# firstBusiness/mathmap

Hardware: AMD Instinct MI355X
Metric: Mpixels/sec (mandelbrot @8192x8192) (higher is better)
Workload: dtype f32

## Files before the change

### mathmap_amd/csrc/hipgen.cpp

```cpp
#include <cmath>
#include <cstdio>
#include <cstdlib>
#include <cstring>
#include <map>
#include <set>
#include <sstream>
#include <stdexcept>

#include "front.h"
#include "hipgen_internal.h"

namespace mm {
namespace hipgen {

std::optional<int> env_int(const char *name) {
    const char *e = getenv(name);
    return e ? std::optional<int>(atoi(e)) : std::nullopt;
}

std::string vname(const Value *v) {
    char buf[64];
    snprintf(buf, sizeof buf, "v%d_%d", v->var->id, v->index);
    return buf;
}
// ... 581 lines not shown
                ok = true;
                bool any_row = false;
                for (const Primary &p : r.args) {
                    ok = ok && operand_ok(p) && (p.kind != Primary::Val || p.value->index < 0 || row_scalar(p.value->var->type));
                    any_row = any_row || (p.kind == Primary::Val && rows.count(p.value));
                }
                ok = ok && any_row && strncmp(r.op->cname, "USERVAL_", 8) != 0;
            }
            if (!ok) continue;
            cand.push_back(s);
            rows.insert(s->lhs);
        }
        std::set<Value *> used;
        for (bool changed = true; changed;) {
            changed = false;
            for (Stmt *s : cand) s->in_pixel = !rows.count(s->lhs);
            std::vector<Value *> defs;
            used.clear();
            collect_values(code.body, PIXEL, defs, used);
            for (int i = 0; i < 4; ++i) used.insert(code.result[i]);
            for (Stmt *s : cand) {
                if (!rows.count(s->lhs)) continue;
                bool drop = used.count(s->lhs) && s->lhs->var->type == Ty::Complex;
                if (s->rhs.kind == Rhs::Prim) drop = drop || !rows.count(s->rhs.prim.value);
                for (const Primary &p : s->rhs.args)
                    drop = drop || (p.kind == Primary::Val && p.value->index >= 0 && !p.value->hoisted && !rows.count(p.value));
                if (drop) { rows.erase(s->lhs); changed = true; }
            }
        }
        bool expensive = false;
        for (Stmt *s : cand)
            expensive = expensive || (rows.count(s->lhs) && s->rhs.kind == Rhs::Op && row_expensive(s->rhs.op->cname));
        for (Stmt *s : cand) if (rows.count(s->lhs) && used.count(s->lhs)) row_transfer.push_back(s->lhs);
        if (!expensive || row_transfer.empty() || row_transfer.size() > 24) {
            for (Stmt *s : cand) s->in_pixel = true;
            row_transfer.clear();
            return;
        }
        for (Stmt *s : cand)
            if (rows.count(s->lhs)) { s->in_row = true; s->in_pixel = false; s->lhs->row_const = true; }
        ks.row_values = (int)row_transfer.size();
        ks.rows_name = "mm_rows";
    }
    void transfer_loads(const std::set<Value *> *only, const char *ind = "  ") {
        for (Value *v : transfer_order)
            if (!only || only->count(v))
                out << ind << "const " << ctype(v->var) << " " << vname(v) << " = *(const " << ctype(v->var) << " *)(XY + " << transfer_off[v] << ");\n";
    }
    void row_loads(const std::string &ind, const char *row) {
        for (size_t k = 0; k < row_transfer.size(); ++k) {
            Value *v = row_transfer[k];
            const std::string at = "A.rowtab[" + std::to_string(k) + " * A.num_rows + " + row + "]";
            out << ind << "const " << ctype(v->var) << " " << vname(v) << " = "
                << (v->var->type == Ty::Int ? "__float_as_int(" + at + ")" : at) << ";\n";
        }
    }

    void analyze_and_layout() {
        find_natives(code.body);
        ks.native_sites = (int)ks.natives.size();
        bool any_in_loop = false;
        for (const NativeCall &nc : ks.natives) any_in_loop = any_in_loop || nc.in_loop;
        NativeCall dynamic_entry;
        dynamic_entry.dynamic = true;
        if (any_in_loop) ks.natives.insert(ks.natives.end(), MM_NATIVE_DYN_CALLS, dynamic_entry);
        ks.direct_native = find_direct_native();
        find_row_slice();
        collect_values(code.body, PROLOGUE, pro_defs, pro_uses);
        collect_values(code.body, PIXEL, pix_defs, pix_uses);
        collect_values(code.body, ROWS, row_defs, row_uses);
        for (Value *v : row_uses) if (v && v->hoisted) pix_uses.insert(v);
        for (int i = 0; i < 4; ++i) pix_uses.insert(code.result[i]);
        std::set<Value *> pix_def_set(pix_defs.begin(), pix_defs.end());
        for (Value *v : row_transfer) pix_def_set.insert(v);
        int off = 0;
        for (NativeCall &nc : ks.natives) {
            nc.record_offset = off;
            off += MM_NATIVE_REC_BYTES;
        }
        if (!ks.natives.empty()) {
            ks.native_ctr_offset = off;
            off += 16;
        }
        for (Value *v : pro_defs) {
            if (!pix_uses.count(v) || pix_def_set.count(v) || transfer_off.count(v)) continue;
            int sz = type_size(v->var);
            int align = sz >= 8 ? 8 : 4;
            off = (off + align - 1) / align * align;
            transfer_off[v] = off;
            transfer_order.push_back(v);
            off += sz;
        }
        if (ks.native_sites < (int)ks.natives.size())
            each_stmt(code.body, [&](const Stmt *s) {
                if (s->kind != Stmt::While || !s->hoisted || !s->in_pixel) return true;
                off = (off + 3) / 4 * 4;
                dual_base_off[s] = off;
                off += 4;
                return false;
            });
        ks.xy_bytes = (off + 15) / 16 * 16;
        if (ks.xy_bytes == 0) ks.xy_bytes = 16;
        ks.has_prologue = !pro_defs.empty();
        for (Value *v : pix_uses)
            if (v && v->index >= 0 && !pix_def_set.count(v) && !transfer_off.count(v))
                throw CompileError("internal: value " + vname(v) + " used in the pixel kernel but defined nowhere");
        pixel_stats(code.body, pixel_stmts, pixel_fetches);
    }

    void run() {
        analyze_and_layout();
        emit_options();
        emit_preludes();
        emit_functions();
        if (pair) pair->emit_helpers();
        emit_prologue_kernel();
        if (ks.row_values > 0) emit_rows_kernel();
        if (opt.sampled) emit_sampled_pixel_kernel();
        else if (opt.shutter) emit_shutter_pixel_kernel();
        else emit_pixel_kernel();
        ks.source = out.str();
        if (opt.variant()) {
            std::string text, key;
            clip_kernel_source(ks, &text, &key);
            ks.source = std::move(text);
            ks.clip_splices.clear();
        }
        ks.key = text_key(ks.source);
        ks.wrapping_ints = opt.edge_x >= 2 || opt.edge_y >= 2;
    }

    void emit_options() {
        int tw = knobs.tile_w.value_or(opt.tile_w);
        if (tw != 8 && tw != 16 && tw != 32 && tw != 64 && tw != 128 && tw != 256) tw = auto_tile_w();
        ks.tile_w = tw;
        ks.tile_h = 256 / tw;
        out << "#define MM_NT_STORE " << knobs.nt_store.value_or(pixel_fetches > 0) << "\n";
        ks.xcd_order = knobs.xcd_order.value_or(2);
        out << "#define MM_XCD_ORDER " << ks.xcd_order << "\n";
        if (knobs.pair_masks) out << "#define MM_PAIR_MASKS " << *knobs.pair_masks << "\n";
        if (knobs.no_same_taps) out << "#define MM_NO_SAME_TAPS 1\n";
        if (knobs.no_outside_shortcut) out << "#define MM_NO_OUTSIDE_SHORTCUT 1\n";
        out << "#define MM_INTERSAMPLE " << opt.intersample << "\n";
        out << "#define MM_SUPERSAMPLING " << opt.supersampling << "\n";
        out << "#define MM_EDGE_X " << opt.edge_x << "\n#define MM_EDGE_Y " << opt.edge_y << "\n";
        if (opt.pixel_inc > 1) out << "#define MM_PIXEL_INC " << opt.pixel_inc << "\n";
        out << "#define MM_TILE_W " << ks.tile_w << "\n#define MM_TILE_H " << ks.tile_h << "\n";
        ks.unroll = opt.unroll > 0 ? opt.unroll : auto_unroll();
        if (opt.variant()) ks.unroll = 1;
        else if (opt.unroll <= 0 && !knobs.unroll && ks.row_values == 0 && ks.natives.empty())
            pair = make_pair_mode(PairEnv{out, code, opt, knobs, pix_defs, pixel_stmts, pixel_fetches,
                                          [this](const Primary &p) { return prim(p, PIXEL); },
                                          [this](const Stmt *s) { return rhs(s->rhs, PIXEL, s, s->lhs->var); },
                                          [this](const Value *v) { return value_visible(v, PIXEL); }});
        if (pair) ks.unroll = 2;
        ks.pair_mode = pair != nullptr;
        ks.pair_exit = pair && pair->exit_driven();
        out << "#define MM_UNROLL " << ks.unroll << "\n";
        out << "#define MM_NATIVE_REC_BYTES " << (int)MM_NATIVE_REC_BYTES << "\n#define MM_NATIVE_DYN_CALLS " << (int)MM_NATIVE_DYN_CALLS << "\n";
    }

    void emit_preludes() {
        out << "#define MMF_FN static __device__ __forceinline__\n#define MMF_CONST_TABLE static __device__ const\n"
               "#define MMG_FN static __device__\n"
               "#define MMF_FMA(a, b, c) __builtin_fma((a), (b), (c))\n#define MMF_RINT(a) __builtin_rint((a))\n"
               "#define MMF_FABSF(a) __builtin_fabsf((a))\n#define MMF_FABS(a) __builtin_fabs((a))\n"
               "#define MMF_SIN_SLOW(a) sin((a))\n#define MMF_COS_SLOW(a) cos((a))\n"
               "#define MMF_LDEXP(a, e) __builtin_ldexp((a), (e))\n#define MMF_EXP_SLOW(a) exp((a))\n#define MMF_LOG_SLOW(a) log((a))\n"
               "#define MMF_POW_SLOW(a, b) pow((a), (b))\n"
               "#define MMF_ASINH_SLOW(a) asinh((a))\n#define MMF_ACOSH_SLOW(a) acosh((a))\n"
               "#define MMF_SQRT(a) __builtin_sqrt((a))\n#define MMF_HYPOT_SLOW(a, b) hypot((a), (b))\n"
               "#define MMQ_FN static __device__ __forceinline__\n#define MMQ_TABLE static __device__ const\n"
               "#define MMQ_FMA(a, b, c) __builtin_fma((a), (b), (c))\n#define MMQ_SQRT(a) sqrt((a))\n"
               "#define MMQ_SQRTF(a) sqrtf((a))\n"
            << device_fastmath_prelude() << "\n";
        out << device_prelude() << "\n";
        bool noise = uses_noise(code.body);
        for (auto &fn : (fn_root ? fn_root : &code)->functions) noise = noise || uses_noise(fn->body);
        if (noise) {
            if (!noise_table_text())
                throw CompileError("the noise builtins need libnoise's gradient table, which was not available when this "
                                   "library was built (see tools/extract_noise_table.py)");
            out << noise_table_text() << device_noise_prelude() << "\n";
        }
        out << R"(
MM_DEV mm_image mm_closure_image(const mm_args &A, int closure_id) {
    mm_image im; im.idx = closure_id < 0 ? -1 : -2 - closure_id; im.pw = A.img_width; im.ph = A.img_height;
    im.xf = im.yf = 1.0f; im.resized = 0; return im;
}
struct mm_narg_t { int kind; int i; float f; mm_image img; };
MM_DEV mm_narg_t mm_narg(int v) { mm_narg_t a; a.kind = 0; a.i = v; a.f = (float)v; a.img = mm_null_image(); return a; }
MM_DEV mm_narg_t mm_narg(float v) { mm_narg_t a; a.kind = 1; a.i = (int)v; a.f = v; a.img = mm_null_image(); return a; }
MM_DEV mm_narg_t mm_narg(double v) { return mm_narg((float)v); }
MM_DEV mm_narg_t mm_narg(mm_image v) { mm_narg_t a; a.kind = 2; a.i = v.idx; a.f = 0.0f; a.img = v; return a; }
// Records a native-filter call for the host (which runs the filter's kernels between
// the prologue and the pixel kernel) and returns the handle of its result float map.
// ctr[0] counts the calls of this frame in the order they are made (the host runs them in that order).
MM_DEV mm_image mm_native_call(const mm_args &A, char *rec, int *ctr, int k, int nargs, mm_narg_t a0, mm_narg_t a1, mm_narg_t a2, mm_narg_t a3) {
    int *hdr = (int *)rec;
    hdr[0] = 1; hdr[1] = k; hdr[2] = nargs; hdr[3] = ctr[0]++;
    mm_narg_t *args = (mm_narg_t *)(rec + 16);
    args[0] = a0; args[1] = a1; args[2] = a2; args[3] = a3;
    mm_image im; im.idx = A.native_slot_base + k; im.pw = A.render_width; im.ph = A.render_height;
    im.xf = im.yf = 1.0f; im.resized = 0;
    return im;
}
// The same for a call site inside a loop: every call takes the next of the MM_NATIVE_DYN_CALLS dynamic entries behind
// the `sites' call sites (record, result slot); one call too many raises ctr[2] and the host refuses the frame.
MM_DEV mm_image mm_native_call_in_loop(const mm_args &A, char *dyn, int *ctr, int site, int sites, int nargs, mm_narg_t a0, mm_narg_t a1,
                                       mm_narg_t a2, mm_narg_t a3) {
    int n = ctr[1]++;
    if (n >= MM_NATIVE_DYN_CALLS) { ctr[2] = 1; n = MM_NATIVE_DYN_CALLS - 1; }
    mm_image im = mm_native_call(A, dyn + n * MM_NATIVE_REC_BYTES, ctr, site, nargs, a0, a1, a2, a3);
    im.idx = A.native_slot_base + sites + n;
    return im;
}
// (float) frame column / row of the pixel being evaluated (render_image's per-pixel loop, builtins.c:324-333)
#define __colF ((float)(col + A.region_x))
#define __rowF ((float)(rl + A.first_row))
#define MM_INTERNALS \
    const float t = A.t; const float R = A.R; const int frame = A.frame; \
    const int __canvasPixelW = A.img_width, __canvasPixelH = A.img_height; \
    const int __renderPixelW = A.render_width, __renderPixelH = A.render_height; \
    (void)t; (void)R; (void)frame; (void)__canvasPixelW; (void)__canvasPixelH; (void)__renderPixelW; (void)__renderPixelH;
)";
        if (ks.native_sites < (int)ks.natives.size())
            out << R"(// The pixel slice's side of a loop that runs in both slices: its n-th call from an in-loop site is the prologue's n-th.
MM_DEV mm_image mm_native_result_in_loop(const mm_args &A, int &n, int sites) {
    mm_image im; im.idx = A.native_slot_base + sites + (n < MM_NATIVE_DYN_CALLS ? n : MM_NATIVE_DYN_CALLS - 1); ++n;
    im.pw = A.render_width; im.ph = A.render_height; im.xf = im.yf = 1.0f; im.resized = 0;
    return im;
}
)";
    }

    void emit_functions() {
        FilterCode &root = fn_root ? *fn_root : code;
        if (root.functions.empty()) return;
        out << "#ifndef MM_MAX_CALL_DEPTH\n#define MM_MAX_CALL_DEPTH " << knobs.max_call_depth.value_or(16)
            << "\n#endif\n"
               "struct mm_uvarg { int i; float f; color_t c; mm_image img; };\n";
        auto head = [](size_t k) {
            return "template <int MM_D> __device__ __noinline__ mm_tup<4> mm_filter_" + std::to_string(k) +
                   "(const mm_args &A, const mm_uvarg *UV, float x, float y, float t, int col, int rl, unsigned &mm_rand_ctr)";
        };
        for (size_t k = 0; k < root.functions.size(); ++k) out << head(k) << ";\n";
        for (size_t k = 0; k < root.functions.size(); ++k) {
            FilterCode &fn = *root.functions[k];
            Generator g(fn, opt, knobs);
            g.fn_root = &root;
            g.in_function = true;
            std::vector<Value *> defs;
            std::set<Value *> uses;
            g.collect_values(fn.body, PIXEL, defs, uses);
            out << "// filter_" << (fn.filter ? fn.filter->name : "") << "\n" << head(k) << " {\n"
                   "  mm_tup<4> rt;\n  rt.v[0] = rt.v[1] = rt.v[2] = rt.v[3] = 0.0f;\n"
                   "  if constexpr (MM_D >= MM_MAX_CALL_DEPTH) { return rt; } else {\n"
                   "  const float R = A.R; const int frame = 0;      // new_template.c.in:379: filter_$name has `int frame = 0`\n"
                   "  const int __canvasPixelW = A.img_width, __canvasPixelH = A.img_height;\n"
                   "  const int __renderPixelW = A.render_width, __renderPixelH = A.render_height;\n"
                   "  (void)R; (void)frame; (void)__canvasPixelW; (void)__canvasPixelH; (void)__renderPixelW; (void)__renderPixelH;\n";
            g.decls(defs, "  ");
            g.stmts(fn.body, PIXEL, "  ");
            out << g.out.str();
            for (int i = 0; i < 4; ++i) out << "  rt.v[" << i << "] = " << g.prim(Primary::V(fn.result[i]), PIXEL) << ";\n";
            out << "  return rt;\n  }\n}\n";
        }
    }

    void emit_prologue_kernel() {
        ks.prologue_uses_time = hoisted_uses_time(code.body);
        ks.prologue_name = "mm_prologue";
        ks.pixel_name = "mm_pixels";
        auto tables = [](const std::string &first) {
            return "  {\n    const int gid = blockIdx.x * 256 + threadIdx.x;\n"
                   "    if (" + first + "gid < A.region_width) A.xtab[gid] = CALC_VIRTUAL_X(gid + A.region_x, A.frame_render_width, A.sampling_offset_x);\n"
                   "    if (" + first + "gid < A.num_rows) A.ytab[gid] = CALC_VIRTUAL_Y(A.first_row + gid, A.frame_render_height, A.sampling_offset_y);\n"
                   "    if (gid != 0) return;\n  }\n";
        };
        const std::string sampled_tables =
            "  {\n    const int gid = blockIdx.x * 256 + threadIdx.x;\n"
            "    if (fi == 0 && gid < A.region_width) {\n"
            "      A.xtab[gid] = CALC_VIRTUAL_X(gid + A.region_x, A.frame_render_width, A.sampling_offset_x);\n"
            "      for (int mm_a = 0; mm_a < S.gx; ++mm_a)\n"
            "        S.xtabs[mm_a * A.region_width + gid] = CALC_VIRTUAL_X(gid + A.region_x, A.frame_render_width, S.offs[mm_a]);\n"
            "    }\n"
            "    if (fi == 0 && gid < A.num_rows) {\n"
            "      A.ytab[gid] = CALC_VIRTUAL_Y(A.first_row + gid, A.frame_render_height, A.sampling_offset_y);\n"
            "      for (int mm_b = 0; mm_b < S.gy; ++mm_b)\n"
            "        S.ytabs[mm_b * A.num_rows + gid] = CALC_VIRTUAL_Y(A.first_row + gid, A.frame_render_height, S.offs[MM_SAMPLE_GRID_MAX + mm_b]);\n"
            "    }\n"
            "    if (gid != 0) return;\n  }\n";
        const std::string clip_head =
            opt.sampled ? std::string(clip_prelude()) + sampled_prelude() + KERNEL +
                              "mm_prologue_clip(mm_args A, char *XY, const mm_clip C, const mm_sampled S) {\n  MM_CLIP_ENTRY\n" + sampled_tables
                        : (ks.natives.empty() ? clip_prelude() : clip_prelude_natives()) + KERNEL +
                              "mm_prologue_clip(mm_args A, char *XY, const mm_clip C) {\n  MM_CLIP_ENTRY\n" + tables("fi == 0 && ");
        emit(KERNEL + "mm_prologue(mm_args A, char *XY) {\n" + tables(""), clip_head);
        out << "  MM_INTERNALS\n";
        if (!(fn_root ? fn_root : &code)->functions.empty()) out << "  const int col = 0, rl = 0; unsigned mm_rand_ctr = 0; (void)col; (void)rl; (void)mm_rand_ctr;\n";
        decls(pro_defs, "  ", true);
        if (!ks.natives.empty()) {
            for (const NativeCall &nc : ks.natives) out << "  *(int *)(XY + " << nc.record_offset << ") = 0;\n";
            out << "  { int *mm_ctr = (int *)(XY + " << ks.native_ctr_offset << "); mm_ctr[0] = mm_ctr[1] = mm_ctr[2] = mm_ctr[3] = 0; }\n";
        }
        stmts(code.body, PROLOGUE, "  ");
        for (Value *v : transfer_order)
// ... 337 lines not shown
```

### mathmap_amd/csrc/hipgen_internal.h

```cpp
#pragma once
#include <functional>
#include <memory>
#include <optional>
#include <ostream>
#include <string>
#include <vector>

#include "hipgen.h"

namespace mm {
namespace hipgen {

enum Slice { PROLOGUE, PIXEL, ROWS };

std::optional<int> env_int(const char *name);
struct Knobs {
    std::optional<int> unroll = env_int("MMHIP_UNROLL");
    std::optional<int> tile_w = env_int("MMHIP_TILE_W");
    std::optional<int> single_pixel = env_int("MMHIP_SINGLE_PIXEL");
    std::optional<int> pair = env_int("MMHIP_PAIR");
    bool pair_debug = env_int("MMHIP_PAIR_DEBUG").has_value();
    std::optional<int> pair_masks = env_int("MMHIP_PAIR_MASKS");
    std::optional<int> pair_exit = env_int("MMHIP_PAIR_EXIT");
    std::optional<int> pair_exit_tail = env_int("MMHIP_PAIR_EXIT_TAIL");
    std::optional<int> pair_pack = env_int("MMHIP_PAIR_PACK");
    std::optional<int> pair_peel = env_int("MMHIP_PAIR_PEEL");
    std::optional<int> pair_fma2 = env_int("MMHIP_PAIR_FMA2");
    std::optional<int> pair_step = env_int("MMHIP_PAIR_STEP");
    bool pair_no_uniform = env_int("MMHIP_PAIR_NO_UNIFORM").has_value();
    std::optional<int> nt_store = env_int("MMHIP_NT_STORE");
    std::optional<int> xcd_order = env_int("MMHIP_XCD_ORDER");
    std::optional<int> waves_per_eu = env_int("MMHIP_WAVES_PER_EU");
    bool no_fetched_result = env_int("MMHIP_NO_FETCHED_RESULT").has_value();
    bool no_same_taps = env_int("MMHIP_NO_SAME_TAPS").has_value();
    bool no_outside_shortcut = env_int("MMHIP_NO_OUTSIDE_SHORTCUT").has_value();
    std::optional<int> frame_hot = env_int("MMHIP_FRAME_HOT");
    bool no_row_slice = env_int("MMHIP_NO_ROW_SLICE").has_value();
    std::optional<int> max_call_depth = env_int("MMHIP_MAX_CALL_DEPTH");
};

std::string vname(const Value *v);
std::string ctype(const CompVar *v);
int type_size(const CompVar *v);
std::string float_literal(float f);
const char *libm_name(const char *cname, bool f32);
bool is_truth_op(const char *cname);
bool is_pow2_divisor(float c);
bool nonneg_or_nan(const Value *v, int depth);
const Primary *sqrt_less_pow2(const Rhs &r, float *kk);

struct PairEnv {
    std::ostream &out;
    FilterCode &code;
    const KernelOptions &opt;
    const Knobs &knobs;
    const std::vector<Value *> &pix_defs;
    int pixel_stmts, pixel_fetches;
    std::function<std::string(const Primary &)> prim;
    std::function<std::string(const Stmt *)> rhs;
    std::function<bool(const Value *)> value_visible;
};
struct PairMode {
    virtual ~PairMode() {}
    virtual bool exit_driven() const = 0;
    virtual bool is_uniform(const Value *v) const = 0;
    virtual void emit_helpers() = 0;
    virtual void emit_pixel_loop(const std::string &ind) = 0;
};
std::unique_ptr<PairMode> make_pair_mode(const PairEnv &env);

}
}
```

### mathmap_amd/csrc/hipgen_pair.cpp

```cpp
#include <algorithm>
#include <cstdio>
#include <cstring>
#include <map>
#include <set>
#include <sstream>

#include "hipgen_internal.h"

namespace mm {
namespace hipgen {
namespace {

struct PairGen final : PairMode {
    PairEnv env;
    std::ostream &out;
    FilterCode &code;
    std::set<const Value *> defs;
    std::set<const Value *> bools;
    std::set<const Value *> uniform;
    int ids = 0;
    const bool exit = env.knobs.pair_exit.value_or(1) && env.knobs.pair_masks.value_or(1);
    const bool pack = exit && env.knobs.pair_pack.value_or(1);
    const Stmt *split_def = nullptr;
    bool split_leave = false;
    const bool fma2 = exit && env.knobs.pair_fma2.value_or(1) && env.knobs.pair_exit_tail.value_or(2) >= 2;
    struct Fuse { const Stmt *r, *d; Primary t, b; float k; bool keep_d; };
    std::map<const Stmt *, std::vector<Fuse>> fuse_plan;
    std::map<const Stmt *, const Fuse *> fusing;
    std::set<const Stmt *> fused_away;
    const bool step = fma2 && pack && !env.knobs.pair_peel.value_or(0) && env.knobs.pair_step.value_or(1);
    bool fast_step = false;
    std::vector<std::string> entry_masks;

    explicit PairGen(const PairEnv &e) : env(e), out(e.out), code(e.code) {}

    bool exit_driven() const override { return exit; }
    bool is_uniform(const Value *v) const override { return uniform.count(v) > 0; }

    static bool scalar_ty(Ty t) { return t == Ty::Int || t == Ty::Float; }
    static bool prim_ok(const Primary &p) {
        if (p.kind == Primary::IntConst || p.kind == Primary::FloatConst) return true;
        return p.kind == Primary::Val && scalar_ty(p.value->var->type);
    }
    static bool rhs_ok(const Rhs &r) {
        if (r.kind == Rhs::Prim) return prim_ok(r.prim);
        if (r.kind == Rhs::Internal) return r.internal == "x" || r.internal == "y";
        if (r.kind != Rhs::Op) return false;
        static const char *ok[] = {"ADD", "SUB", "MUL", "NEG", "DIV", "LESS", "LEQ", "EQ", "NOT", "sqrt"};
        bool found = false;
        for (const char *o : ok) found = found || !strcmp(r.op->cname, o);
        if (!found) return false;
        for (const Primary &a : r.args) if (!prim_ok(a)) return false;
        if (!strcmp(r.op->cname, "sqrt") && r.args[0].type() != Ty::Float) return false;
        if (!strcmp(r.op->cname, "NOT") && r.args[0].type() != Ty::Int) return false;
        return true;
    }
    bool block_ok(const Block &b) const {
        for (const Stmt *s : b) {
            if (!s->in_pixel) continue;
            switch (s->kind) {
                case Stmt::Assign:
                    if (!s->lhs || !scalar_ty(s->lhs->var->type) || !rhs_ok(s->rhs)) {
                        if (env.knobs.pair_debug)
                            fprintf(stderr, "pair mode: statement not covered (%s)\n",
                                    s->rhs.kind == Rhs::Op ? s->rhs.op->cname : s->rhs.kind == Rhs::Internal ? s->rhs.internal.c_str() : "rhs kind");
                        return false;
                    }
                    break;
                case Stmt::If:
                case Stmt::While:
                    if (s->cond.kind != Rhs::Prim || !prim_ok(s->cond.prim) || s->cond.prim.type() != Ty::Int) return false;
                    for (const Stmt *ph : s->phis) {
                        if (!ph->in_pixel) continue;
                        if (!scalar_ty(ph->lhs->var->type) || ph->rhs.kind != Rhs::Prim || ph->rhs2.kind != Rhs::Prim ||
                            !prim_ok(ph->rhs.prim) || !prim_ok(ph->rhs2.prim))
                            return false;
                    }
                    if (s->kind == Stmt::If ? !(block_ok(s->then_) && block_ok(s->else_)) : !block_ok(s->body)) return false;
                    break;
                default: break;
            }
        }
        return true;
    }
    bool eligible() const {
        if (!env.opt.fast_math_exact) return false;
        const bool force = env.knobs.pair.has_value();
        if (force && !*env.knobs.pair) return false;
        const int stmts = env.pixel_stmts;
        if (env.pixel_fetches || stmts < 4 || stmts > (force ? 400 : 40)) return false;
        const bool dbg = env.knobs.pair_debug;
        for (int i = 0; i < 4; ++i)
            if (!code.result[i] || !scalar_ty(code.result[i]->var->type)) {
                if (dbg) fprintf(stderr, "pair mode: result %d is not an int / float value\n", i);
                return false;
            }
        const bool ok = block_ok(code.body);
        if (dbg) fprintf(stderr, "pair mode: body %s (%d statements)\n", ok ? "covered" : "not covered", stmts);
        return ok;
    }

    template <class P> static bool truth_def(const Stmt *d, P operand) {
        if (d->kind == Stmt::Phi) return d->rhs.kind == Rhs::Prim && d->rhs2.kind == Rhs::Prim && operand(d->rhs.prim) && operand(d->rhs2.prim);
        if (d->kind != Stmt::Assign) return false;
        if (d->rhs.kind == Rhs::Prim) return operand(d->rhs.prim);
        return d->rhs.kind == Rhs::Op && is_truth_op(d->rhs.op->cname);
    }
    static bool const_is_bool(const Value *v, int depth) {
        if (!v || depth > 12 || v->var->type != Ty::Int) return false;
        if (v->index < 0) return true;
        return v->def && truth_def(v->def, [&](const Primary &p) {
            return p.kind == Primary::IntConst ? p.i == 0 || p.i == 1 : p.kind == Primary::Val && const_is_bool(p.value, depth + 1);
        });
    }
    bool prim_bool(const Primary &p) const {
        if (p.kind == Primary::IntConst) return p.i == 0 || p.i == 1;
        if (p.kind != Primary::Val) return false;
        if (p.value->index < 0) return p.value->var->type == Ty::Int;
        if (bools.count(p.value)) return true;
        return !defs.count(p.value) && const_is_bool(p.value, 0);
    }
    void infer_bools() {
        std::vector<const Stmt *> idefs;
        for (Value *v : env.pix_defs) {
            defs.insert(v);
            if (v->var->type == Ty::Int && v->def && v->def->lhs == v) idefs.push_back(v->def);
        }
        for (const Stmt *d : idefs) bools.insert(d->lhs);
        for (bool changed = true; changed;) {
            changed = false;
            for (const Stmt *d : idefs)
                if (bools.count(d->lhs) && !truth_def(d, [&](const Primary &p) { return prim_bool(p); })) { bools.erase(d->lhs); changed = true; }
        }
    }
    void uses_outside(const Block &b, const Stmt *skip, std::set<const Value *> &uses) const {
        auto use = [&](const Primary &p) { if (p.kind == Primary::Val) uses.insert(p.value); };
        auto use_rhs = [&](const Rhs &r) { if (r.kind == Rhs::Prim) use(r.prim); for (const Primary &a : r.args) use(a); };
        for (const Stmt *s : b) {
            if (!s->in_pixel) continue;
            if (s->kind == Stmt::Assign) use_rhs(s->rhs);
            if (s->kind == Stmt::If) {
                use_rhs(s->cond);
                uses_outside(s->then_, skip, uses);
                uses_outside(s->else_, skip, uses);
                for (const Stmt *ph : s->phis) if (ph->in_pixel) { use_rhs(ph->rhs); use_rhs(ph->rhs2); }
            }
            if (s->kind == Stmt::While) {
                for (const Stmt *ph : s->phis) if (ph->in_pixel) { use_rhs(ph->rhs); if (s != skip) use_rhs(ph->rhs2); }
                if (s != skip) { use_rhs(s->cond); uses_outside(s->body, skip, uses); }
            }
        }
    }

    std::string pbool(const Primary &p) {
        const std::string bu = exit ? "mm_xbu(" : "mm_bu(";
        if (p.kind == Primary::IntConst) return bu + (p.i ? "true)" : "false)");
        if (p.kind == Primary::Val && p.value->index < 0) return bu + "false)";
        if (uniform.count(p.value)) return "mm_bu((bool)u" + vname(p.value) + ")";
        if (bools.count(p.value)) return vname(p.value);
        if (fast_step && !defs.count(p.value)) {
            const std::string c = env.prim(p);
            size_t k = std::find(entry_masks.begin(), entry_masks.end(), c) - entry_masks.begin();
            if (k == entry_masks.size()) entry_masks.push_back(c);
            return "mm_ub" + std::to_string(k);
        }
        return "mm_tob(" + pprim(p, Ty::Int) + ")";
    }
    std::string pprim(const Primary &p, Ty want) {
        const char *w = want == Ty::Float ? "mm_vf(" : "mm_vi(";
        if (p.kind == Primary::IntConst) return std::string(w) + std::to_string(p.i) + ")";
        if (p.kind == Primary::FloatConst) return std::string(w) + float_literal(p.f) + "f)";
        if (p.value->index < 0) return std::string(w) + "0)";
        if (uniform.count(p.value))
            return std::string(w) + (p.value->var->type == Ty::Float ? "(float)u" : "(int)u") + vname(p.value) + ")";
        return std::string(w) + vname(p.value) + ")";
    }
    static Ty arith_ty(const Rhs &r) {
        for (const Primary &a : r.args) if (a.type() == Ty::Float) return Ty::Float;
        return Ty::Int;
    }
    std::string prhs(const Rhs &r, const Value *lhs) {
        const Ty lhs_ty = lhs->var->type;
        const bool as_bool = bools.count(lhs) > 0;
        if (r.kind == Rhs::Prim) return as_bool ? pbool(r.prim) : pprim(r.prim, lhs_ty);
// ... 585 lines not shown
                                << pval_as(ph->rhs2.prim, ph->lhs) << ");\n";
                    break;
                }
                case Stmt::While: while_loop(s, ind, mask); break;
                default: break;
            }
        }
    }

    void emit_helpers() override {
        if (exit)
            out << R"(#define MM_PAIR_EXIT 1
// exit-driven pair loops (hipgen.cpp pair_while_exit).  mm_xnotb: a lane mask's bits outside exec are never read -- selects
// read their own lane's bit, and every mask a branch tests is ANDed with one that lies inside exec -- so NOT needs no re-AND
// and a broadcast no ballot.
MM_DEV mm_bb mm_xnotb(mm_bb a) { return mm_bb{~a.x, ~a.y}; }
MM_DEV mm_bb mm_xbu(bool u) { const unsigned long m = u ? ~0ul : 0ul; return mm_bb{m, m}; }      // a literal truth value, likewise
// a wave-uniform int for the exit copies, moved from its scalar register where it is wanted (as an ordinary operand it
// would pull the loop counter, and the loop's bound test, onto the vector unit)
MM_DEV int mm_s2v(int u) { int r; asm("v_mov_b32 %0, %1" : "=v"(r) : "s"(__builtin_amdgcn_readfirstlane(u))); return r; }
)";
        bool guarded = false;
        for (const auto &lp : fuse_plan) for (const Fuse &f : lp.second) guarded = guarded || needs_guard(f.b);
        if (guarded)
            out << R"(#define MM_PAIR_FMA2 1
// fused doubling (hipgen_pair.cpp plan_fusion): fl(fl(t * 2^k) + b) is fma(t, 2^k, b) -- the product is exact -- unless the
// product overflows and the exact sum does not, which takes |b| > 2^103.  True when no lane of the wave holds such an
// addend in either pixel (NaN fails the comparison): the loop then runs in its fused copy.
MM_DEV bool mm_fma2_ok(mm_pf b) {
  return __builtin_amdgcn_ballot_w64(!(__builtin_fabsf(b.x) <= 0x1p102f && __builtin_fabsf(b.y) <= 0x1p102f)) == 0ul;
}
)";
        if (fast_step)
            out << R"(#define MM_PAIR_STEP 1
// the fast pair step (hipgen_pair.cpp emit_pixel_loop): a step that lies inside the launch's rows addresses the y table and the
// output as a wave-uniform 64-bit base -- the tile's first row -- plus a 32-bit lane offset that follows mm_p.  The offset is
// formed next to the access, so base and offset go into the instruction's own saddr form: no 64-bit vector arithmetic is left.
MM_DEV mm_pf mm_load_y2(const char *sy, unsigned oy) {      // both rows' y, one 8-byte load (the offset is a multiple of 8)
  typedef float mm_y2v __attribute__((ext_vector_type(2)));
  const mm_y2v y = *(const mm_y2v *)(sy + oy);
  return mm_pf{y.x, y.y};
}
// a frame constant read as a truth value: wave-uniform, so its lane mask is all ones or zero and is made on the scalar unit, once,
// in front of the pixel loop.  Bits outside exec are set: mm_xnotb's argument covers it (selects read their own lane's bit, and
// the mask a loop tests is ANDed with mm_bu(true), which lies inside exec).  (Through a scalar register by name: a select between
// 64-bit constants on a uniform bool is a v_cndmask_b32 pair to this compiler.)
MM_DEV mm_bb mm_xbs(int u) {
  unsigned long m = (unsigned long)(long)__builtin_amdgcn_readfirstlane(u != 0 ? -1 : 0);
  asm("" : "+s"(m));
  return mm_bb{m, m};
}
)";
        emit_store_pair();
    }

    struct Pack {
        std::vector<const Value *> vals;
        int src[4];
        float lit[4];
    };
    static bool literal_of(const Value *v, float &f, int depth = 0) {
        if (!v || depth > 8) return false;
        if (v->index < 0) { f = 0; return true; }
        const Stmt *d = v->def;
        if (!d || d->kind != Stmt::Assign || d->lhs != v || d->rhs.kind != Rhs::Prim) return false;
        const Primary &p = d->rhs.prim;
        if (p.kind == Primary::IntConst) { f = (float)p.i; return true; }
        if (p.kind == Primary::FloatConst) { f = p.f; return v->var->type == Ty::Float && f == f; }
        return p.kind == Primary::Val && p.value->var->type == v->var->type && literal_of(p.value, f, depth + 1);
    }
    bool plan_pack(Pack &pk) const {
        if (!pack) return false;
        for (int i = 0; i < 4; ++i) {
            const Value *v = code.result[i];
            pk.src[i] = -1;
            if (literal_of(v, pk.lit[i])) continue;
            const auto it = std::find(pk.vals.begin(), pk.vals.end(), v);
            pk.src[i] = (int)(it - pk.vals.begin());
            if (it == pk.vals.end()) pk.vals.push_back(v);
        }
        return !pk.vals.empty();
    }
    void emit_store_pair() {
        Pack pk;
        if (!plan_pack(pk)) return;
        const int n = (int)pk.vals.size();
        unsigned k = 0;
        for (int i = 0; i < 4; ++i)
            if (pk.src[i] < 0) {
                const float c = pk.lit[i] < 0.0f ? 0.0f : pk.lit[i] > 1.0f ? 1.0f : pk.lit[i];
                k |= (unsigned)(255.0 * (double)c) << (8 * i);
            }
        auto sel = [&](int second, int first) {
            unsigned s = 0;
            for (int i = 0; i < 4; ++i) s |= (pk.src[i] == second && second >= 0 ? 0x00u : pk.src[i] == first && first >= 0 ? 0x04u : 0x0cu) << (8 * i);
            return s;
        };
        auto hex = [](unsigned v) { char b[16]; snprintf(b, sizeof b, "0x%08xu", v); return std::string(b); };
        auto word = [&](const char *px) {
            auto u = [&](int j) { return std::string("u") + px + std::to_string(j); };
            if (n == 1) {
                unsigned s1 = 0;
                for (int i = 0; i < 4; ++i) s1 |= (pk.src[i] == 0 ? 0x04u : (unsigned)i) << (8 * i);
                return "__builtin_amdgcn_perm(" + u(0) + ", " + hex(k) + ", " + hex(s1) + ")";
            }
            std::string w = "__builtin_amdgcn_perm(" + u(1) + ", " + u(0) + ", " + hex(sel(0, 1)) + ")";
            if (n > 2) w += " | __builtin_amdgcn_perm(" + (n > 3 ? u(3) : u(2)) + ", " + u(2) + ", " + hex(sel(2, n > 3 ? 3 : -1)) + ")";
            return k ? w + " | " + hex(k) : w;
        };
        auto convert = [&](const char *I) {
            out << I;
            for (int j = 0; j < n; ++j) out << " a" << j << " = mm_clamp01(a" << j << "); b" << j << " = mm_clamp01(b" << j << ");";
            out << "\n" << I << " unsigned";
            for (int j = 0; j < n; ++j) out << (j ? ", " : " ") << "ua" << j << ", ub" << j;
            out << ";\n" << I << " asm volatile(\"s_setreg_imm32_b32 hwreg(HW_REG_MODE, 0, 2), 3\\n\\t\"\n";
            for (int j = 0; j < 2 * n; ++j) out << I << "              \"v_fma_f32 %" << j << ", %" << 2 * n + j << ", %" << 4 * n << ", %" << 4 * n + 1 << "\\n\\t\"\n";
            out << I << "              \"s_setreg_imm32_b32 hwreg(HW_REG_MODE, 0, 2), 0\"\n" << I << "              :";
            for (int j = 0; j < n; ++j) out << (j ? ", " : " ") << "\"=&v\"(ua" << j << "), \"=&v\"(ub" << j << ")";
            out << "\n" << I << "              :";
            for (int j = 0; j < n; ++j) out << " \"v\"(a" << j << "), \"v\"(b" << j << "),";
            out << " \"s\"(255.0f), \"v\"(8388608.0f));\n";
        };
        out << "// this kernel's result pack (hipgen_pair.cpp emit_store_pair): both pixels of a step, " << n << " distinct value" << (n > 1 ? "s" : "")
            << " per pixel, literal bytes " << hex(k) << "\n"
            << "MM_DEV void mm_store_pair(const mm_args &A, int row_a, int row_b, int col";
        for (int j = 0; j < n; ++j) out << ", float a" << j << ", float b" << j;
        out << ") {\n  if (__builtin_expect(!A.floatmap && A.output_bpp == 4, 1)) {\n";
        convert("   ");
        out << "    MM_STORE_U32((unsigned *)((unsigned char *)A.out + (long)row_a * A.row_stride + (long)col * 4), " << word("a") << ");\n"
            << "    MM_STORE_U32((unsigned *)((unsigned char *)A.out + (long)row_b * A.row_stride + (long)col * 4), " << word("b") << ");\n"
            << "    return;\n  }\n  mm_tup<4> ra, rb;\n";
        for (int i = 0; i < 4; ++i) {
            if (pk.src[i] < 0) out << "  ra.v[" << i << "] = rb.v[" << i << "] = " << float_literal(pk.lit[i]) << "f;\n";
            else out << "  ra.v[" << i << "] = a" << pk.src[i] << "; rb.v[" << i << "] = b" << pk.src[i] << ";\n";
        }
        out << "  mm_store_pixel(A, row_a, col, ra);\n  mm_store_pixel(A, row_b, col, rb);\n}\n";
        if (!fast_step) return;
        out << "// the same words from a fast step (mm_load_y2, above): `so` the step's first output row, oa / ob this lane's offsets in its two rows\n"
            << "MM_DEV void mm_store_step(unsigned char *so, unsigned oa, unsigned ob";
        for (int j = 0; j < n; ++j) out << ", float a" << j << ", float b" << j;
        out << ") {\n";
        convert(" ");
        out << "  MM_STORE_U32((unsigned *)(so + oa), " << word("a") << ");\n"
            << "  MM_STORE_U32((unsigned *)(so + ob), " << word("b") << ");\n}\n";
    }
    void emit_pixel_loop(const std::string &I) override {
        Pack pk;
        const bool packed = plan_pack(pk);
        if (fast_step) {
            std::ostringstream body;
            std::streambuf *const own = out.rdbuf(body.rdbuf());
            emit_steps(I, pk, packed);
            out.rdbuf(own);
            out << I << "// the fast step (hipgen_pair.cpp emit_pixel_loop): decided once; this lane's offsets from the tile's first row, that row's wave-uniform bases\n"
                << I << "const bool mm_fast = !A.floatmap && A.output_bpp == 4 && A.row_stride >= 0 && ((MM_TILE_H * A.ppt) & 1) == 0 && ((unsigned long)A.ytab & 7ul) == 0ul &&\n"
                << I << "                     (long)(MM_TILE_H * (A.ppt + 1) - 1) * A.row_stride + (long)A.region_width * 4 <= 0xffffffffl;\n"
                << I << "const unsigned mm_tr = threadIdx.x / MM_TILE_W;\n"
                << I << "const unsigned mm_oa = (unsigned)col * 4u + 2u * mm_tr * (unsigned)A.row_stride, mm_ob = mm_oa + (unsigned)A.row_stride, mm_oy = 8u * mm_tr;\n"
                << I << "const unsigned mm_ss = (unsigned)(MM_TILE_H * A.row_stride);      // mm_p counts rows MM_TILE_H apart\n"
                << I << "const int mm_sr = __builtin_amdgcn_readfirstlane(tile_y * (MM_TILE_H * A.ppt));\n"
                << I << "unsigned char *const mm_so = (unsigned char *)A.out + (long)mm_sr * A.row_stride;\n"
                << I << "const char *const mm_sy = (const char *)(A.ytab + mm_sr);\n"
                << I << "// the steps, in mm_p, that lie inside the launch's rows (none: not a launch for the fast step): one scalar compare per step\n"
                << I << "const int mm_pin = mm_fast ? (A.num_rows - mm_sr) / (2 * MM_TILE_H) * 2 : 0;\n"
                << I << "// (a copy per test: one truth value read in several places would live across branches, which this compiler keeps as a lane\n"
                << I << "// mask -- s_cselect_b64, s_and_b64 with exec, a branch on vcc -- and an if / else on it goes through a flag block; four one-sided\n"
                << I << "// tests of scalars the compiler takes for unrelated are s_cmp and a branch on scc each)\n"
                << I << "int mm_pin_a = mm_pin, mm_pin_b = mm_pin, mm_pin_c = mm_pin;\n"
                << I << "asm(\"\" : \"+s\"(mm_pin_a), \"+s\"(mm_pin_b), \"+s\"(mm_pin_c));\n";
            for (size_t k = 0; k < entry_masks.size(); ++k)
                out << I << "const mm_bb mm_ub" << k << " = mm_xbs(" << entry_masks[k] << ");\n";
            out << body.str();
            return;
        }
        emit_steps(I, pk, packed);
    }
    void emit_steps(const std::string &I, const Pack &pk, bool packed) {
        const std::string E = fast_step ? I + "  " : I;
        out << "#pragma unroll 1\n" << I << "for (; mm_p < A.ppt; mm_p += 2) {\n";
        if (fast_step)
            out << I << "  const bool mm_in = mm_p < mm_pin;      // wave-uniform: the fast step is for this launch and the whole step lies inside its rows\n"
                << I << "  mm_pf mm_y2;\n"
                << I << "  if (__builtin_expect(mm_in, 1)) mm_y2 = mm_load_y2(mm_sy, mm_oy + (unsigned)mm_p * (4u * MM_TILE_H));\n"
                << I << "  if (__builtin_expect(mm_p >= mm_pin_a, 0)) {      // (!mm_in) the step as it was\n";
        out << E << "  // vertically adjacent pixels: they mostly take the same path (a wave covers 16 x 8 pixels per step)\n"
            << E << "  const int rl_a = row0 + (int)(threadIdx.x / MM_TILE_W) + mm_p * MM_TILE_H, rl_b = rl_a + 1;\n"
            << E << "  const int row_a = rl_a < A.num_rows ? rl_a : A.num_rows - 1, row_b = rl_b < A.num_rows ? rl_b : A.num_rows - 1;\n"
            << E << (fast_step ? "  mm_y2 = mm_pf{A.ytab[row_a], A.ytab[row_b]};" : "  const mm_pf mm_y2 = {A.ytab[row_a], A.ytab[row_b]};") << "    // CALC_VIRTUAL_Y per row, by the prologue\n";
        if (fast_step) out << I << "  }\n";
        std::set<Value *> seen;
        for (Value *v : env.pix_defs)
            if (v->index >= 0 && seen.insert(v).second) out << I << "  " << pair_ctype(v) << " " << vname(v) << ";\n";
        stmts(code.body, I + "  ", "mm_bu(true)");
        if (packed) {
            std::string vals;
            for (const Value *v : pk.vals) {
                const std::string e = pprim(Primary::V(const_cast<Value *>(v)), Ty::Float);
                vals += ", " + e + ".x, " + e + ".y";
            }
            if (fast_step)
                out << I << "  if (__builtin_expect(mm_p < mm_pin_b, 1)) {      // (mm_in)\n"
                    << I << "    const unsigned mm_sp = (unsigned)mm_p * mm_ss;\n"
                    << I << "    mm_store_step(mm_so, mm_oa + mm_sp, mm_ob + mm_sp" << vals << ");\n"
                    << I << "  }\n"
                    << I << "  if (__builtin_expect(mm_p >= mm_pin_c, 0)) {      // (!mm_in) the step as it was\n"
                    << E << "  const int rl_a = row0 + (int)(threadIdx.x / MM_TILE_W) + mm_p * MM_TILE_H, rl_b = rl_a + 1;\n"
                    << E << "  const int row_a = rl_a < A.num_rows ? rl_a : A.num_rows - 1, row_b = rl_b < A.num_rows ? rl_b : A.num_rows - 1;\n";
            out << E << "  // a row past the end was evaluated as the last row: storing it there again writes the same bytes\n"
                << E << "  mm_store_pair(A, row_a, row_b, col" << vals << ");\n";
            if (fast_step)
                out << I << "  }\n";
            out << I << "}\n";
            return;
        }
        out << I << "  mm_tup<4> mm_ra, mm_rb;\n";
        for (int i = 0; i < 4; ++i) {
            const std::string v = pprim(Primary::V(code.result[i]), Ty::Float);
            out << I << "  mm_ra.v[" << i << "] = " << v << ".x; mm_rb.v[" << i << "] = " << v << ".y;\n";
        }
        out << I << "  // a row past the end was evaluated as the last row: storing it there again writes the same bytes\n"
            << I << "  mm_store_pixel(A, row_a, col, mm_ra);\n"
            << I << "  mm_store_pixel(A, row_b, col, mm_rb);\n" << I << "}\n";
    }
};

}

std::unique_ptr<PairMode> make_pair_mode(const PairEnv &env) {
    std::unique_ptr<PairGen> g(new PairGen(env));
    if (!g->eligible()) return nullptr;
    g->infer_bools();
    g->plan_fusion();
    PairGen::Pack pk;
    g->fast_step = g->step && !g->fuse_plan.empty() && g->plan_pack(pk);
    return g;
}

}
}
```

Baseline: 429,900.

## Spread pair-mode steps across tile rows so workgroups interleave segments

Adds a 'spread' mode, on by default, that changes how the fast pair step assigns rows to workgroups. Instead of each workgroup covering one contiguous block of MM_TILE_H*ppt rows, segment k of a workgroup takes step k*mm_nty+tile_y, walking the launch's rows with a stride. Per-segment bases move by one scalar addition each, and an asm barrier keeps the lane offsets in 32-bit vector registers for saddr addressing. This is meant to even out work across workgroups, since Mandelbrot cost varies by region and contiguous blocks can leave some workgroups with far more iterations. It also adds an emit_both callback, presumably emitting both a clipped and an unclipped variant.

```diff
diff --git a/mathmap_amd/csrc/hipgen.cpp b/mathmap_amd/csrc/hipgen.cpp
--- a/mathmap_amd/csrc/hipgen.cpp
+++ b/mathmap_amd/csrc/hipgen.cpp
@@ -757,7 +757,8 @@
             pair = make_pair_mode(PairEnv{out, code, opt, knobs, pix_defs, pixel_stmts, pixel_fetches,
                                           [this](const Primary &p) { return prim(p, PIXEL); },
                                           [this](const Stmt *s) { return rhs(s->rhs, PIXEL, s, s->lhs->var); },
-                                          [this](const Value *v) { return value_visible(v, PIXEL); }});
+                                          [this](const Value *v) { return value_visible(v, PIXEL); },
+                                          [this](const std::string &text, const std::string &clip_text) { emit(text, clip_text); }});
         if (pair) ks.unroll = 2;
         ks.pair_mode = pair != nullptr;
         ks.pair_exit = pair && pair->exit_driven();
diff --git a/mathmap_amd/csrc/hipgen_internal.h b/mathmap_amd/csrc/hipgen_internal.h
--- a/mathmap_amd/csrc/hipgen_internal.h
+++ b/mathmap_amd/csrc/hipgen_internal.h
@@ -27,6 +27,7 @@
     std::optional<int> pair_peel = env_int("MMHIP_PAIR_PEEL");
     std::optional<int> pair_fma2 = env_int("MMHIP_PAIR_FMA2");
     std::optional<int> pair_step = env_int("MMHIP_PAIR_STEP");
+    std::optional<int> pair_spread = env_int("MMHIP_PAIR_SPREAD");
     bool pair_no_uniform = env_int("MMHIP_PAIR_NO_UNIFORM").has_value();
     std::optional<int> nt_store = env_int("MMHIP_NT_STORE");
     std::optional<int> xcd_order = env_int("MMHIP_XCD_ORDER");
@@ -59,6 +60,7 @@
     std::function<std::string(const Primary &)> prim;
     std::function<std::string(const Stmt *)> rhs;
     std::function<bool(const Value *)> value_visible;
+    std::function<void(const std::string &, const std::string &)> emit_both;
 };
 struct PairMode {
     virtual ~PairMode() {}
diff --git a/mathmap_amd/csrc/hipgen_pair.cpp b/mathmap_amd/csrc/hipgen_pair.cpp
--- a/mathmap_amd/csrc/hipgen_pair.cpp
+++ b/mathmap_amd/csrc/hipgen_pair.cpp
@@ -30,6 +30,7 @@
     std::set<const Stmt *> fused_away;
     const bool step = fma2 && pack && !env.knobs.pair_peel.value_or(0) && env.knobs.pair_step.value_or(1);
     bool fast_step = false;
+    bool spread = false;
     std::vector<std::string> entry_masks;
 
     explicit PairGen(const PairEnv &e) : env(e), out(e.out), code(e.code) {}
@@ -921,25 +922,77 @@
             std::streambuf *const own = out.rdbuf(body.rdbuf());
             emit_steps(I, pk, packed);
             out.rdbuf(own);
-            out << I << "// the fast step (hipgen_pair.cpp emit_pixel_loop): decided once; this lane's offsets from the tile's first row, that row's wave-uniform bases\n"
-                << I << "const bool mm_fast = !A.floatmap && A.output_bpp == 4 && A.row_stride >= 0 && ((MM_TILE_H * A.ppt) & 1) == 0 && ((unsigned long)A.ytab & 7ul) == 0ul &&\n"
-                << I << "                     (long)(MM_TILE_H * (A.ppt + 1) - 1) * A.row_stride + (long)A.region_width * 4 <= 0xffffffffl;\n"
-                << I << "const unsigned mm_tr = threadIdx.x / MM_TILE_W;\n"
-                << I << "const unsigned mm_oa = (unsigned)col * 4u + 2u * mm_tr * (unsigned)A.row_stride, mm_ob = mm_oa + (unsigned)A.row_stride, mm_oy = 8u * mm_tr;\n"
-                << I << "const unsigned mm_ss = (unsigned)(MM_TILE_H * A.row_stride);      // mm_p counts rows MM_TILE_H apart\n"
-                << I << "const int mm_sr = __builtin_amdgcn_readfirstlane(tile_y * (MM_TILE_H * A.ppt));\n"
-                << I << "unsigned char *const mm_so = (unsigned char *)A.out + (long)mm_sr * A.row_stride;\n"
-                << I << "const char *const mm_sy = (const char *)(A.ytab + mm_sr);\n"
-                << I << "// the steps, in mm_p, that lie inside the launch's rows (none: not a launch for the fast step): one scalar compare per step\n"
-                << I << "const int mm_pin = mm_fast ? (A.num_rows - mm_sr) / (2 * MM_TILE_H) * 2 : 0;\n"
-                << I << "// (a copy per test: one truth value read in several places would live across branches, which this compiler keeps as a lane\n"
-                << I << "// mask -- s_cselect_b64, s_and_b64 with exec, a branch on vcc -- and an if / else on it goes through a flag block; four one-sided\n"
-                << I << "// tests of scalars the compiler takes for unrelated are s_cmp and a branch on scc each)\n"
-                << I << "int mm_pin_a = mm_pin, mm_pin_b = mm_pin, mm_pin_c = mm_pin;\n"
-                << I << "asm(\"\" : \"+s\"(mm_pin_a), \"+s\"(mm_pin_b), \"+s\"(mm_pin_c));\n";
+            auto lane_head = [](const std::string &I, const char *offsets) {
+                return I + "// the fast step (hipgen_pair.cpp emit_pixel_loop): decided once; this lane's offsets from the tile's first row, that row's wave-uniform bases\n" +
+                       I + "const bool mm_fast = !A.floatmap && A.output_bpp == 4 && A.row_stride >= 0 && ((MM_TILE_H * A.ppt) & 1) == 0 && ((unsigned long)A.ytab & 7ul) == 0ul &&\n" +
+                       I + "                     (long)(MM_TILE_H * (A.ppt + 1) - 1) * A.row_stride + (long)A.region_width * 4 <= 0xffffffffl;\n" +
+                       I + "const unsigned mm_tr = threadIdx.x / MM_TILE_W;\n" +
+                       I + offsets + " mm_oa = (unsigned)col * 4u + 2u * mm_tr * (unsigned)A.row_stride, mm_ob = mm_oa + (unsigned)A.row_stride, mm_oy = 8u * mm_tr;\n" +
+                       I + "const unsigned mm_ss = (unsigned)(MM_TILE_H * A.row_stride);      // mm_p counts rows MM_TILE_H apart\n";
+            };
+            auto row_head = [](const std::string &I, const std::string &sr) {
+                return I + "const int mm_sr = __builtin_amdgcn_readfirstlane(" + sr + ");\n" +
+                       I + "unsigned char *const mm_so = (unsigned char *)A.out + (long)mm_sr * A.row_stride;\n" +
+                       I + "const char *const mm_sy = (const char *)(A.ytab + mm_sr);\n" +
+                       I + "// the steps, in mm_p, that lie inside the launch's rows (none: not a launch for the fast step): one scalar compare per step\n" +
+                       I + "const int mm_pin = mm_fast ? (A.num_rows - mm_sr) / (2 * MM_TILE_H) * 2 : 0;\n";
+            };
+            auto pin_copies = [](const std::string &I) {
+                return I + "// (a copy per test: one truth value read in several places would live across branches, which this compiler keeps as a lane\n" +
+                       I + "// mask -- s_cselect_b64, s_and_b64 with exec, a branch on vcc -- and an if / else on it goes through a flag block; four one-sided\n" +
+                       I + "// tests of scalars the compiler takes for unrelated are s_cmp and a branch on scc each)\n" +
+                       I + "int mm_pin_a = mm_pin, mm_pin_b = mm_pin, mm_pin_c = mm_pin;\n" +
+                       I + "asm(\"\" : \"+s\"(mm_pin_a), \"+s\"(mm_pin_b), \"+s\"(mm_pin_c));\n";
+            };
+            std::string masks;
             for (size_t k = 0; k < entry_masks.size(); ++k)
-                out << I << "const mm_bb mm_ub" << k << " = mm_xbs(" << entry_masks[k] << ");\n";
-            out << body.str();
+                masks += I + "const mm_bb mm_ub" + std::to_string(k) + " = mm_xbs(" + entry_masks[k] + ");\n";
+            const std::string steps = body.str();
+            const std::string tile = lane_head(I, "const unsigned") + row_head(I, "tile_y * (MM_TILE_H * A.ppt)") + pin_copies(I) + masks + steps;
+            if (!spread) {
+                out << tile;
+                return;
+            }
+            const std::string J = I + "  ", E = I + "    ";
+            auto replace_all = [](std::string s, const std::string &was, const std::string &is) {
+                for (size_t at = s.find(was); at != std::string::npos; at = s.find(was, at + is.size())) s.replace(at, was.size(), is);
+                return s;
+            };
+            const std::string rows_was = E + "const int rl_a = row0 + ";
+            const std::string seg = replace_all(replace_all(steps, "for (; mm_p < A.ppt; mm_p += 2) {\n", "for (mm_p = 0; mm_p < 2; mm_p += 2) {      // one step per segment\n"), rows_was,
+                                                E + "int row0 = mm_sr;      // the segment's first row, not the tile's\n" +
+                                                E + "asm volatile(\"\" : \"+s\"(row0));\n" +
+                                                E + "row0 += (int)(threadIdx.x / MM_TILE_W);\n" + rows_was);
+            std::string body_in;
+            for (size_t b = 0, e; b < seg.size(); b = e + 1) {
+                e = seg.find('\n', b);
+                if (e == std::string::npos) e = seg.size() - 1;
+                body_in += (seg[b] == '#' || seg[b] == '\n' ? "" : "  ") + seg.substr(b, e + 1 - b);
+            }
+            env.emit_both(lane_head(I, "unsigned") + masks +
+                              I + "// spread steps (hipgen_pair.cpp emit_pixel_loop): segment k of this workgroup is step k * mm_nty + tile_y of the launch's rows\n" +
+                              I + "const int mm_nty = (A.tiles_magic ? (int)__umulhi((unsigned)(nwg - 1), A.tiles_magic) : (nwg - 1) / tiles_x) + 1;      // the launch's tile rows\n" +
+                              I + "// the first segment: its first row, the bases there, the whole steps (times two) from that row to the launch's last\n" +
+                              row_head(I, "tile_y * (2 * MM_TILE_H)") +
+                              I + "// from segment to segment all of them move by mm_nty steps -- one scalar addition each, nothing is multiplied or divided per\n" +
+                              I + "// step -- up to the workgroup's last segment or the launch's last row: a segment that starts at or past it has nothing to do\n" +
+                              I + "const int mm_ds = mm_nty * (2 * MM_TILE_H), mm_last = mm_sr + (A.ppt >> 1) * mm_ds, mm_end = mm_last < A.num_rows ? mm_last : A.num_rows;\n" +
+                              I + "const long mm_dso = (long)mm_ds * A.row_stride;\n" +
+                              I + "int mm_srk = mm_sr, mm_pink = mm_pin;\n" +
+                              I + "unsigned char *mm_sok = mm_so;\n" +
+                              I + "const char *mm_syk = mm_sy;\n" +
+                              "#pragma nounroll\n" +
+                              I + "for (; mm_srk < mm_end; mm_srk += mm_ds, mm_sok += mm_dso, mm_syk += 4 * mm_ds, mm_pink -= 2 * mm_nty) {\n" +
+                              J + "const int mm_sr = mm_srk, mm_pin = mm_pink;      // this segment's, under the names the step knows\n" +
+                              J + "unsigned char *const mm_so = mm_sok;\n" +
+                              J + "const char *const mm_sy = mm_syk;\n" +
+                              pin_copies(J) +
+                              J + "// (the lane offsets no longer change from step to step: left to itself the compiler adds them to the frame's base once, as\n" +
+                              J + "// 64-bit vector addresses, and adds the segment's distance to those per step -- the saddr form, a scalar base and these\n" +
+                              J + "// 32-bit offsets, needs no vector instruction at all)\n" +
+                              J + "asm volatile(\"\" : \"+v\"(mm_oa), \"+v\"(mm_ob), \"+v\"(mm_oy));\n" +
+                              body_in + I + "}\n",
+                          tile);
             return;
         }
         emit_steps(I, pk, packed);
@@ -1002,6 +1055,7 @@
     g->plan_fusion();
     PairGen::Pack pk;
     g->fast_step = g->step && !g->fuse_plan.empty() && g->plan_pack(pk);
+    g->spread = g->fast_step && env.knobs.pair_spread.value_or(1);
     return g;
 }
 
```

Result: faster. 437,400 (median of 6 runs) (+1.7%).
